# zwu88/TANTE

Hardware: AMD Instinct MI355X
Metric: rollout frames/sec (fwd), TANTE on 256x256 Active Matter (higher is better)
Workload: dtype bf16

## Files before the change

### tante_amd/_lib.py

```python
import ctypes as C
import os

HERE = os.path.dirname(os.path.abspath(__file__))
LIB_PATH = os.environ.get("TANTE_LIB") or os.path.join(HERE, "lib", "libtante_hip.so")

F32, BF16 = 0, 1
INSTNORM_INSTANCE, INSTNORM_RMS = 0, 1
ACT_NONE, ACT_GELU_ERF, ACT_GELU_TANH, ACT_RELU = 0, 1, 2, 3
A_LINEAR, A_PATCH_NHWC, A_PATCH_NCHW = 0, 1, 2
E_LINEAR, E_FILM, E_DECONV_NHWC, E_DECONV_NCHW = 0, 1, 2, 3
W_LINEAR, W_CONV_NHWC, W_DECONV_NHWC, W_DECONV_NCHW = 0, 1, 2, 3
W_LINEAR_T, W_CONV_NHWC_T, W_DECONV_NHWC_T, W_DECONV_NCHW_T = 4, 5, 6, 7

c_i32, c_i64, c_f32, c_vp = C.c_int32, C.c_int64, C.c_float, C.c_void_p


class PackGeom(C.Structure):
    _fields_ = [("n_pad", c_i32), ("k_pad", c_i32), ("nt", c_i32), ("cb", c_i32), ("bytes", c_i64)]


class Gemm(C.Structure):
    _fields_ = [
        ("a", c_vp), ("a_dtype", c_i32), ("a_mode", c_i32), ("M", c_i32), ("K", c_i32),
        ("a_s1", c_i64), ("a_s0", c_i64), ("a_off", c_i64), ("a_n0", c_i32),
# ... 222 lines not shown
    "tante_attention_flash_masked": ([c_vp, c_vp, c_vp, c_i32, c_i32, c_i32, c_i32, c_i32, c_i32, c_vp, c_i64, c_vp, c_f32, C.c_uint64, c_vp], c_i32),
    "tante_attention_flash_masked_bwd": ([c_vp, c_vp, c_vp, c_vp, c_vp, c_i32, c_i32, c_i32, c_i32, c_i32, c_i32, c_vp, c_i64, c_vp, c_f32, C.c_uint64, c_vp], c_i32),
    "tante_head_enc_supported": ([c_i32, c_i32], c_i32),
    "tante_head_enc_stream_bytes": ([c_i32], c_i64),
    "tante_head_enc_ws_bytes": ([c_i64], c_i64),
    "tante_pack_head_enc": ([c_vp] * 6 + [c_i32, c_i32, c_vp, c_vp], c_i32),
    "tante_head_enc_fused": ([c_i32, c_vp, c_vp, c_vp, c_i32, c_i64, c_i64, c_i64, c_i32, c_i32, c_i32, c_i32, c_i32, c_vp, c_i64, c_vp, c_i64,
                             c_vp, c_vp, c_vp, c_i64, c_vp], c_i32),
    "tante_adaptive_tail_supported": ([c_i32] * 6, c_i32),
    "tante_adaptive_rt_stream_bytes": ([c_i32], c_i64),
    "tante_adaptive_ws_bytes": ([c_i32, c_i32, c_i32, c_i32], c_i64),
    "tante_pack_adaptive_rt": ([c_vp] * 6 + [c_i32, c_vp, c_vp], c_i32),
    "tante_adaptive_rt": ([c_i32, c_vp, c_vp, c_vp, c_i32, c_i64, c_i64, c_i64, c_i32, c_i32, c_i32, c_i32, c_f32, c_f32, c_vp, c_i64,
                           c_vp, c_vp, c_vp, c_vp, c_vp, c_vp], c_i32),
    "tante_head_adaptive": ([c_i32, c_vp, c_vp, c_i32, c_i64, c_i64, c_i64, c_i32, c_i32, c_i32, c_i32, c_i32, c_vp, c_vp, c_vp, c_i32, c_vp,
                             c_i32, c_vp, c_i64, c_vp, c_i64, c_vp], c_i32),
    "tante_afno_filter_supported": ([c_i64, c_i32, c_i32, c_i32, c_i32], c_i32),
    "tante_afno_twiddle_floats": ([c_i32, c_i32], c_i64),
    "tante_afno_filter_workspace_bytes": ([c_i64, c_i32, c_i32, c_i32], c_i64),
    "tante_afno_filter": ([c_vp, c_vp, c_i64, c_i32, c_i32, c_i32, c_i32, c_vp, c_vp, c_vp, c_f32, c_vp, c_vp, c_i64, c_vp], c_i32),
    "tante_afno_twiddle_bwd_floats": ([c_i32, c_i32], c_i64),
    "tante_afno_filter_bwd_workspace_bytes": ([c_i64, c_i32, c_i32, c_i32, c_i32], c_i64),
    "tante_afno_filter_bwd": ([c_vp, c_vp, c_i64, c_i32, c_i32, c_i32, c_i32, c_vp, c_vp, c_vp, c_vp, c_f32, c_vp, c_vp, c_vp, c_i32, c_vp, c_vp,
                               c_i64, c_vp], c_i32),
    "tante_groupnorm_supported": ([c_i64, c_i32, c_i32, c_i32], c_i32),
    "tante_groupnorm_workspace_bytes": ([c_i64, c_i32, c_i32, c_i32], c_i64),
    "tante_groupnorm": ([c_vp, c_i64, c_i32, c_i32, c_i32, c_f32, c_vp, c_vp, c_vp, c_i32, c_vp, c_i64, c_vp], c_i32),
    "tante_dpot_filter_supported": ([c_i64, c_i32, c_i32, c_i32, c_i32, c_i32, c_i32], c_i32),
    "tante_dpot_twiddle_floats": ([c_i32, c_i32, c_i32], c_i64),
    "tante_dpot_filter_workspace_bytes": ([c_i64, c_i32, c_i32, c_i32, c_i32, c_i32], c_i64),
    "tante_dpot_filter": ([c_vp, c_vp, c_i64, c_i32, c_i32, c_i32, c_i32, c_i32, c_i32, c_vp, c_vp, c_vp, c_vp, c_vp, c_vp, c_vp, c_i64, c_vp],
                          c_i32),
    "tante_groupnorm_bwd_supported": ([c_i64, c_i32, c_i32, c_i32], c_i32),
    "tante_groupnorm_bwd_workspace_bytes": ([c_i64, c_i32, c_i32, c_i32], c_i64),
    "tante_groupnorm_bwd": ([c_vp, c_i32, c_vp, c_i64, c_i32, c_i32, c_i32, c_f32, c_vp, c_vp, c_vp, c_vp, c_i32, c_vp, c_i64, c_vp], c_i32),
    "tante_dpot_twiddle_bwd_floats": ([c_i32, c_i32, c_i32], c_i64),
    "tante_dpot_filter_bwd_workspace_bytes": ([c_i64, c_i32, c_i32, c_i32, c_i32, c_i32], c_i64),
    "tante_dpot_filter_bwd": ([c_vp, c_vp, c_i64, c_i32, c_i32, c_i32, c_i32, c_i32, c_vp, c_vp, c_vp, c_vp, c_vp, c_vp, c_vp, c_vp, c_vp, c_vp,
                               c_i32, c_vp, c_i64, c_vp], c_i32),
    "tante_instnorm_supported": ([c_i64, c_i32, c_i32], c_i32),
    "tante_instnorm_workspace_bytes": ([c_i64, c_i32, c_i32], c_i64),
    "tante_instnorm": ([c_vp, c_i64, c_i32, c_i32, c_i32, c_f32, c_vp, c_vp, c_i32, c_vp, c_vp, c_vp, c_i32, c_vp, c_i64, c_vp], c_i32),
    "tante_axial_attention_supported": ([c_i64, c_i32, c_i32, c_i32, c_i32], c_i32),
    "tante_axial_attention": ([c_vp, c_i64, c_i32, c_i32, c_i32, c_i32, c_vp, c_vp, c_vp, c_vp, c_f32, c_vp, c_vp], c_i32),
    "tante_time_attention_supported": ([c_i64, c_i32, c_i32, c_i32], c_i32),
    "tante_time_attention": ([c_vp, c_i64, c_i32, c_i32, c_i32, c_vp, c_vp, c_vp, c_vp, c_f32, c_vp, c_vp, c_vp], c_i32),
    "tante_field_stats_supported": ([c_i64, c_i32, c_i32, c_i64], c_i32),
    "tante_field_stats_workspace_bytes": ([c_i64, c_i32, c_i32, c_i64], c_i64),
    "tante_field_stats": ([c_vp, c_i64, c_i32, c_i32, c_i64, c_f32, c_vp, c_vp, c_vp, c_i64, c_vp], c_i32),
    "tante_field_affine_supported": ([c_i64, c_i32, c_i32, c_i64], c_i32),
    "tante_field_affine": ([c_vp, c_vp, c_i64, c_i32, c_i32, c_i64, c_vp, c_vp], c_i32),
    "tante_convnext_block_supported": ([c_i64, c_i32, c_i32, c_i32], c_i32),
    "tante_convnext_stream_bytes": ([c_i32], c_i64),
    "tante_pack_convnext": ([c_vp] * 6 + [c_i32, c_i32, c_vp, c_vp], c_i32),
    "tante_convnext_block": ([c_vp, c_vp, c_vp, c_i64, c_i32, c_i32, c_i32, c_i32, c_f32, c_vp], c_i32),
    "tante_dwconv_ln_supported": ([c_i64, c_i32, c_i32, c_i32], c_i32),
    "tante_dwconv_ln": ([c_vp, c_i64, c_i32, c_i32, c_i32, c_vp, c_vp, c_f32, c_vp, c_vp, c_vp, c_i32, c_vp], c_i32),
    "tante_l2norm_rows_supported": ([c_i64, c_i32], c_i32),
    "tante_l2norm_rows": ([c_vp, c_i64, c_i32, c_f32, c_vp, c_i32, c_vp], c_i32),
    "tante_conv3x3_supported": ([c_i64, c_i32, c_i32, c_i32, c_i32], c_i32),
    "tante_conv3x3": ([c_vp, c_i64, c_i32, c_i32, c_i32, c_i32, c_vp, c_vp, c_i32, c_vp, c_i32, c_vp], c_i32),
    "tante_conv3x3_mfma_supported": ([c_i64, c_i32, c_i32, c_i32, c_i32, c_i32, c_i32], c_i32),
    "tante_conv3x3_pack_bytes": ([c_i32, c_i32, c_i32], c_i64),
    "tante_pack_conv3x3": ([c_vp, c_i32, c_i32, c_i32, c_vp, c_vp], c_i32),
    "tante_conv3x3_mfma": ([c_vp, c_i32, c_vp, c_i32, c_i64, c_i32, c_i32, c_i32, c_i32, c_i32, c_vp, c_vp, c_i32, c_i32, c_i32, c_vp, c_i32, c_vp],
                           c_i32),
    "tante_attn_gate_supported": ([c_i64, c_i32, c_i32, c_i32], c_i32),
    "tante_attn_gate_stream_bytes": ([c_i32, c_i32, c_i32, c_i32], c_i64),
    "tante_pack_attn_gate": ([c_vp, c_vp, c_vp, c_f32, c_i32, c_i32, c_i32, c_i32, c_vp, c_vp], c_i32),
    "tante_attn_gate": ([c_vp, c_vp, c_i64, c_i32, c_i32, c_i32, c_vp, c_i32, c_vp, c_vp], c_i32),
    "tante_uno_block_supported": ([c_i64, c_i32, c_i32, c_i32, c_i32, c_i32, c_i32, c_i32, c_i32, c_i64, c_i64], c_i32),
    "tante_uno_table_floats": ([c_i32, c_i32, c_i32, c_i32, c_i32, c_i32, c_i32], c_i64),
    "tante_uno_table_layout": ([c_i32, c_i32, c_i32, c_i32, c_i32, c_i32, c_i32, c_vp], c_i32),
    "tante_uno_block_workspace_bytes": ([c_i64, c_i32, c_i32, c_i32, c_i32, c_i32, c_i32, c_i32, c_i32, c_i32], c_i64),
    "tante_uno_block": ([c_vp, c_i64, c_i64, c_i32, c_i32, c_i32, c_i32, c_i32, c_i32, c_i32, c_i32, c_vp, c_vp, c_vp, c_vp, c_vp, c_i32, c_vp, c_i64,
                         c_vp, c_i64, c_vp], c_i32),
    "tante_uno_mode_mix_supported": ([c_i64, c_i32, c_i32, c_i32, c_i32], c_i32),
    "tante_uno_mode_mix": ([c_vp, c_vp, c_vp, c_vp, c_i64, c_i32, c_i32, c_i32, c_i32, c_vp], c_i32),
}

LIB_OPTIONS = ("TANTE_ATTN_BWD_HG", "TANTE_ATTN_BWD_NO_SPLIT", "TANTE_ATTN_BWD_VALU", "TANTE_ATTN_FWD_VALU", "TANTE_AXIS_BWD_SMALL_WGS",
               "TANTE_AXIS_BLOCKS", "TANTE_AXIS_BWD_WGS", "TANTE_AXIS_CT", "TANTE_AXIS_FILM", "TANTE_AXIS_GENERIC", "TANTE_AXIS_MFMA", "TANTE_AXIS_NT", "TANTE_AXIS_WGRAD_WGS",
               "TANTE_BLOCK_KERNEL", "TANTE_COLSUM_ROWS", "TANTE_CONV3_FORM","TANTE_CVIT_CHAIN_TOKENS", "TANTE_ENC23_SPLIT", "TANTE_FILM_BWD_ROWS",
               "TANTE_FS_GROUPS", "TANTE_FS_HALF", "TANTE_FS_SKEW", "TANTE_FS_WAVES", "TANTE_GEMM_NO_LITE", "TANTE_GEMM_SMALLM", "TANTE_GEMM_WGS", "TANTE_HEAD_WAVES",
               "TANTE_IM2COL_TILED", "TANTE_RAW_ENCODE_ONE_LAUNCH", "TANTE_RESIZE_TILED", "TANTE_SPECTRAL_BF16OUT", "TANTE_SPECTRAL_DFT", "TANTE_SPECTRAL_X3", "TANTE_WGRAD_DEEP",
               "TANTE_WGRAD_JOBS", "TANTE_WGRAD_JOBS_WGS", "TANTE_WGRAD_NO_SLAB", "TANTE_WGRAD_NO_TR", "TANTE_WGRAD_REDUCE_NY",
               "TANTE_WGRAD_RG", "TANTE_WGRAD_SLAB_WGS", "TANTE_WGRAD_TR_WGS", "TANTE_WGRAD_WGS", "TANTE_XATTN_GPW", "TANTE_XATTN_STREAM", "TANTE_XATTN_VALU",)


_lib = None
ABI_VERSION = 14


def lib():
    global _lib
    if _lib is None:
        if not os.path.exists(LIB_PATH):
            raise RuntimeError(
                f"{LIB_PATH} is missing: build it with `python -m tante_amd.build` "
                "(or __graft_entry__.build()).  tante_amd has no CPU / eager fallback.")
        L = C.CDLL(LIB_PATH)
        for name, (argtypes, restype) in SIGNATURES.items():
            fn = getattr(L, name)
            fn.argtypes = argtypes
            fn.restype = restype
        got = int(L.tante_abi_version())
        if got != ABI_VERSION:
            raise RuntimeError(f"{LIB_PATH}: library ABI {got}, this binding expects {ABI_VERSION} -- a stale build (or a stale variant under "
                               "TANTE_LIB); rebuild with `python -m tante_amd.build`")
        _lib = L
        import warnings
        for k in LIB_OPTIONS:
            v = os.environ.get(k)
            if v is None:
                continue
            try:
                rc = L.tante_set_option(k.encode(), int(v))
            except ValueError:
                warnings.warn(f"{k}={v!r}: library options are integers; ignored")
                continue
            if rc != 0:
                warnings.warn(f"{k}={v}: tante_set_option refused it ({L.tante_last_error().decode(errors='replace')})")
    return _lib


def set_option(name: str, value: int) -> None:
    check(lib().tante_set_option(name.encode(), int(value)), "tante_set_option")


def get_option(name: str, default: int = 0) -> int:
    return int(lib().tante_get_option(name.encode(), int(default)))


def check(rc: int, what: str = ""):
    if rc != 0:
        msg = lib().tante_last_error().decode(errors="replace")
        raise RuntimeError(f"libtante_hip {what} failed (rc={rc}): {msg}")
```

### tante_amd/csrc/block_fused.hip

```cpp
#include "common.hip.h"

#include <stdlib.h>
#include "fused_common.hip.h"
#include "block_sliced.h"

namespace {

constexpr int BIAS_BYTES = 4096;

__device__ __forceinline__ long seq_token(const TanteSeq& q, int s, int l) {
  return (long)(s / q.n_s0) * q.S1 + (long)(s % q.n_s0) * q.S0 + (long)(l / q.n_l0) * q.P1 + (long)(l % q.n_l0) * q.P0;
}

template <int BYTES>
__device__ __forceinline__ void glds_copy(const char* __restrict__ g, char* l, int tid) {
  static_assert(BYTES % 4096 == 0, "tiles are whole LDS-DMA passes");
  const int wave = tid >> 6, lane = tid & 63;
#pragma unroll
  for (int i = 0; i < BYTES / 4096; ++i) {
    const int off = i * 4096 + wave * 1024;
    __builtin_amdgcn_global_load_lds((const __attribute__((address_space(1))) void*)(g + off + lane * 16),
                                     (__attribute__((address_space(3))) void*)(l + off), 16, 0, 0);
  }
}
// ... 632 lines not shown
  if (C != 64 && C != 128 && C != 256) return 0;
  if (hidden != C && hidden != 2 * C) return 0;
  if (hidden > 256 && C == 256) return 0;
  if (L <= 0 || L > 32 || 32 % L) return 0;
  return 1;
}

static int64_t block_ts_stream_bytes(int C, int hidden) {
  const long cpr = C / 8, cprh = hidden / 8;
  return (long)(C / 32) * (96 * cpr * 16 + BIAS_BYTES) + (long)(C / 64 + hidden / 64) * (64 * cpr * 16 + BIAS_BYTES) +
         (long)(C / 64) * (64 * cprh * 16 + BIAS_BYTES);
}

static bool use_fs(int C, int n_head, int hidden, int L, int causal) {
  const int which = tante_opt("TANTE_BLOCK_KERNEL", 0);
  if (!tante_fs_supported(C, n_head, hidden, L, causal)) return false;
  return which == 0 || !block_ts_supported(C, n_head, hidden, L);
}

extern "C" int tante_block_fused_supported(int C, int n_head, int hidden, int L) {
  return block_ts_supported(C, n_head, hidden, L) || tante_fs_supported(C, n_head, hidden, L, 0);
}

extern "C" int64_t tante_block_stream_bytes(int C, int hidden) { return block_ts_stream_bytes(C, hidden) + tante_fs_stream_bytes(C, hidden); }

extern "C" int tante_pack_block(const float* ln1_w, const float* ln1_b, const float* in_w, const float* in_b, const float* out_w,
                                const float* out_b, const float* ln2_w, const float* ln2_b, const float* fc1_w,
                                const float* fc1_b, const float* fc2_w, const float* fc2_b, int C, int hidden,
                                void* block_stream, void* stream) {
  if (!ln1_w || !ln1_b || !in_w || !in_b || !out_w || !out_b || !ln2_w || !ln2_b || !fc1_w || !fc1_b || !fc2_w || !fc2_b ||
      !block_stream)
    TANTE_FAIL(-1, "tante_pack_block: null pointer");
  if (!block_ts_supported(C, C / 32, hidden, 32)) TANTE_FAIL(-2, "tante_pack_block: unsupported C=%d hidden=%d", C, hidden);
  hipLaunchKernelGGL(pack_block_stream_kernel, dim3(C / 32 + 2 * (C / 64) + hidden / 64), dim3(256), 0, (hipStream_t)stream, in_w,
                     in_b, ln1_w, ln1_b, out_w, out_b, fc1_w, fc1_b, ln2_w, ln2_b, fc2_w, fc2_b, C, hidden, (char*)block_stream);
  TANTE_CHECK_LAUNCH();
  if (tante_fs_stream_bytes(C, hidden) > 0) {
    tante_fs_pack(ln1_w, ln1_b, in_w, in_b, out_w, out_b, ln2_w, ln2_b, fc1_w, fc1_b, fc2_w, fc2_b,
                  (char*)block_stream + block_ts_stream_bytes(C, hidden), (hipStream_t)stream);
    TANTE_CHECK_LAUNCH();
  }
  return 0;
}

extern "C" int tante_block_fused_tprop(float* x, const void* block_stream, int C, int n_head, int hidden, const TanteSeq* seq, int causal, float eps,
                                       const float* tprop, void* stream) {
  if (!x || !block_stream || !seq || !tprop) TANTE_FAIL(-1, "tante_block_fused_tprop: null pointer");
  if (seq->L != 4 || !tante_block_fused_supported(C, n_head, hidden, seq->L) || !use_fs(C, n_head, hidden, seq->L, causal))
    TANTE_FAIL(-2, "tante_block_fused_tprop: the feature-sliced kernel at L = 4 only (C=%d heads=%d hidden=%d L=%d)", C, n_head, hidden, seq->L);
  if (((uintptr_t)x % 16) || ((uintptr_t)block_stream % 16)) TANTE_FAIL(-1, "tante_block_fused_tprop: buffers must be 16-byte aligned");
  if (tante_fs_launch(x, (const char*)block_stream + block_ts_stream_bytes(C, hidden), *seq, causal, eps, (hipStream_t)stream, nullptr, tprop) != 0)
    TANTE_FAIL(-2, "tante_block_fused_tprop: too many sequences (%d)", seq->nseq);
  TANTE_CHECK_LAUNCH();
  return 0;
}

extern "C" int tante_block_fused_last_supported(int C, int n_head, int hidden, int L) {
  return C == 256 && n_head == 8 && hidden == 256 && L == 4 && use_fs(C, n_head, hidden, L, 0);
}

extern "C" int tante_block_fused_last(float* x, const void* block_stream, int C, int n_head, int hidden, const TanteSeq* seq, int causal,
                                      float eps, const float* tprop, void* stream) {
  if (!x || !block_stream || !seq) TANTE_FAIL(-1, "tante_block_fused_last: null pointer");
  if (!tante_block_fused_last_supported(C, n_head, hidden, seq->L))
    TANTE_FAIL(-2, "tante_block_fused_last: the feature-sliced kernel at C = 256 / 8 heads / hidden 256 / L = 4 only (C=%d heads=%d hidden=%d L=%d)",
               C, n_head, hidden, seq->L);
  if (((uintptr_t)x % 16) || ((uintptr_t)block_stream % 16)) TANTE_FAIL(-1, "tante_block_fused_last: buffers must be 16-byte aligned");
  if (tante_fs_launch(x, (const char*)block_stream + block_ts_stream_bytes(C, hidden), *seq, causal, eps, (hipStream_t)stream, nullptr, tprop,
                      true) != 0)
    TANTE_FAIL(-2, "tante_block_fused_last: too many sequences (%d)", seq->nseq);
  TANTE_CHECK_LAUNCH();
  return 0;
}

extern "C" int tante_block_fused(float* x, const void* block_stream, int C, int n_head, int hidden, const TanteSeq* seq, int causal,
                                 float eps, void* stream) {
  if (!x || !block_stream || !seq) TANTE_FAIL(-1, "tante_block_fused: null pointer");
  if (!tante_block_fused_supported(C, n_head, hidden, seq->L))
    TANTE_FAIL(-2, "tante_block_fused: unsupported shape C=%d heads=%d hidden=%d L=%d", C, n_head, hidden, seq->L);
  if (((uintptr_t)x % 16) || ((uintptr_t)block_stream % 16)) TANTE_FAIL(-1, "tante_block_fused: buffers must be 16-byte aligned");
  hipStream_t s = (hipStream_t)stream;
  const char* st = (const char*)block_stream;
  if (use_fs(C, n_head, hidden, seq->L, causal)) {
    if (tante_fs_launch(x, st + block_ts_stream_bytes(C, hidden), *seq, causal, eps, s) != 0)
      TANTE_FAIL(-2, "tante_block_fused: too many sequences (%d)", seq->nseq);
    TANTE_CHECK_LAUNCH();
    return 0;
  }
  const int key = (C / 32) * 100 + hidden / 32;
  switch (key) {
    case 202: launch_block<2, 2>(x, st, *seq, causal, eps, s); break;
    case 204: launch_block<2, 4>(x, st, *seq, causal, eps, s); break;
    case 404: launch_block<4, 4>(x, st, *seq, causal, eps, s); break;
    case 408: launch_block<4, 8>(x, st, *seq, causal, eps, s); break;
    case 808: launch_block<8, 8>(x, st, *seq, causal, eps, s); break;
    default: TANTE_FAIL(-2, "tante_block_fused: no instantiation for C=%d hidden=%d", C, hidden);
  }
  TANTE_CHECK_LAUNCH();
  return 0;
}

extern "C" int tante_block_fused_train(const float* x, const void* block_stream, int C, int n_head, int hidden, const TanteSeq* seq, int causal,
                                       float eps, const TanteBlockTrain* tr, void* stream) {
  if (!x || !block_stream || !seq || !tr || !tr->out || !tr->xh1 || !tr->o || !tr->xh2 || !tr->hpre || !tr->act || !tr->st1 ||
      !tr->st2)
    TANTE_FAIL(-1, "tante_block_fused_train: null pointer");
  if (!tante_fs_supported(C, n_head, hidden, seq->L, causal) || seq->L > 64)
    TANTE_FAIL(-2, "tante_block_fused_train: unsupported shape C=%d heads=%d hidden=%d L=%d", C, n_head, hidden, seq->L);
  if (tr->p_drop < 0.0f || tr->p_drop >= 1.0f) TANTE_FAIL(-1, "tante_block_fused_train: dropout probability %f", (double)tr->p_drop);
  const char* st = (const char*)block_stream + block_ts_stream_bytes(C, hidden);
  if (tante_fs_launch((float*)x, st, *seq, causal, eps, (hipStream_t)stream, tr) != 0)
    TANTE_FAIL(-2, "tante_block_fused_train: launch refused (L=%d, %d sequences)", seq->L, seq->nseq);
  TANTE_CHECK_LAUNCH();
  return 0;
}

extern "C" int tante_pack_block_train_multi(const TanteBlockWeights* blocks, int n, int C, int hidden, void* stream) {
  if (!blocks || n <= 0) TANTE_FAIL(-1, "tante_pack_block_train_multi: bad argument");
  if (tante_fs_stream_bytes(C, hidden) == 0) TANTE_FAIL(-2, "tante_pack_block_train_multi: unsupported C=%d hidden=%d", C, hidden);
  for (int g = 0; g < n; g += TANTE_FSP_MAX) {
    const int m = n - g < TANTE_FSP_MAX ? n - g : TANTE_FSP_MAX;
    const float* params[TANTE_FSP_MAX][8];
    char* dst[TANTE_FSP_MAX];
    for (int e = 0; e < m; ++e) {
      const TanteBlockWeights& b = blocks[g + e];
      if (!b.in_w || !b.in_b || !b.out_w || !b.out_b || !b.fc1_w || !b.fc1_b || !b.fc2_w || !b.fc2_b || !b.block_stream)
        TANTE_FAIL(-1, "tante_pack_block_train_multi: null pointer in entry %d", g + e);
      const float* q[8] = {b.in_w, b.in_b, b.out_w, b.out_b, b.fc1_w, b.fc1_b, b.fc2_w, b.fc2_b};
      for (int k = 0; k < 8; ++k) params[e][k] = q[k];
      dst[e] = (char*)b.block_stream + block_ts_stream_bytes(C, hidden);
    }
    tante_fs_pack_folded_multi(params, dst, m, (hipStream_t)stream);
  }
  TANTE_CHECK_LAUNCH();
  return 0;
}

extern "C" int tante_pack_block_train(const float* in_w_folded, const float* in_b_folded, const float* out_w, const float* out_b,
                                      const float* fc1_w_folded, const float* fc1_b_folded, const float* fc2_w, const float* fc2_b, int C,
                                      int hidden, void* block_stream, void* stream) {
  if (!in_w_folded || !in_b_folded || !out_w || !out_b || !fc1_w_folded || !fc1_b_folded || !fc2_w || !fc2_b || !block_stream)
    TANTE_FAIL(-1, "tante_pack_block_train: null pointer");
  if (tante_fs_stream_bytes(C, hidden) == 0) TANTE_FAIL(-2, "tante_pack_block_train: unsupported C=%d hidden=%d", C, hidden);
  tante_fs_pack_folded(in_w_folded, in_b_folded, out_w, out_b, fc1_w_folded, fc1_b_folded, fc2_w, fc2_b,
                       (char*)block_stream + block_ts_stream_bytes(C, hidden), (hipStream_t)stream);
  TANTE_CHECK_LAUNCH();
  return 0;
}
```

### tante_amd/csrc/block_sliced.h

```cpp
#pragma once
#include <hip/hip_runtime.h>
#include <stdint.h>
#include "../../include/tante_hip.h"

int tante_fs_supported(int C, int n_head, int hidden, int L, int causal);
int64_t tante_fs_stream_bytes(int C, int hidden);
void tante_fs_pack(const float* ln1_w, const float* ln1_b, const float* in_w, const float* in_b, const float* out_w, const float* out_b,
                   const float* ln2_w, const float* ln2_b, const float* fc1_w, const float* fc1_b, const float* fc2_w,
                   const float* fc2_b, char* dst, hipStream_t s);
void tante_fs_pack_folded(const float* in_w, const float* in_b, const float* out_w, const float* out_b, const float* fc1_w,
                          const float* fc1_b, const float* fc2_w, const float* fc2_b, char* dst, hipStream_t s);
constexpr int TANTE_FSP_MAX = 12;
void tante_fs_pack_folded_multi(const float* const (*params)[8], char* const* dst, int n, hipStream_t s);
int tante_fs_launch(float* x, const char* stream, const TanteSeq& sq, int causal, float eps, hipStream_t s, const TanteBlockTrain* tr = nullptr,
                    const float* tprop = nullptr, bool lastq = false);
```

### tante_amd/csrc/block_sliced.hip

```cpp
#include "common.hip.h"
#include "fused_common.hip.h"
#include "fs_common.hip.h"
#include "block_sliced.h"

namespace {


struct FsArgs {
  float* x;
  const char* w;
  TanteSeq sq;
  int causal;
  float eps;
  int spw;
  unsigned magic;
  float* out;
  unsigned short *xh1, *qkv, *o, *xh2, *hpre, *act;
  float *st1, *x1, *st2;
  float p_drop;
  unsigned long long seed_attn, seed_out, seed_mlp;
  const unsigned long long* seed_mix;
  unsigned long long* stamps;
  const float* tprop;
  int skew;
};

#ifdef TANTE_ABLATE
#define FS_STAMP(k)                                                                                        \
  do {                                                                                                     \
    if (A.stamps) {                                                                                        \
      unsigned long long t_;                                                                               \
      __builtin_amdgcn_sched_barrier(0);                                                                   \
      asm volatile("s_memtime %0\n\ts_waitcnt lgkmcnt(0)" : "=s"(t_)::"memory");                          \
      __builtin_amdgcn_sched_barrier(0);                                                                   \
      if (lane == 0) A.stamps[((long)vblock * 8 + wave) * 20 + (k)] = t_;                               \
    }                                                                                                      \
  } while (0)
unsigned long long* g_fs_stamps = nullptr;
#else
#define FS_STAMP(k)
#endif

__device__ __forceinline__ void fs_divmod(int a, int n, float rn, int& q, int& r) {
  q = (int)((float)a * rn);
  r = a - q * n;
  if (r >= n) { ++q; r -= n; }
  if (r < 0) { --q; r += n; }
}
struct FsSeqMap {
  float rs0, rl0;
  __device__ __forceinline__ explicit FsSeqMap(const TanteSeq& q) : rs0(__builtin_amdgcn_rcpf((float)q.n_s0)), rl0(__builtin_amdgcn_rcpf((float)q.n_l0)) {}
  __device__ __forceinline__ long token(const TanteSeq& q, int s, int l) const {
    int a, b, c, d;
    fs_divmod(s, q.n_s0, rs0, a, b);
    fs_divmod(l, q.n_l0, rl0, c, d);
    return (long)a * q.S1 + (long)b * q.S0 + (long)c * q.P1 + (long)d * q.P0;
  }
};


struct TpropW {
  float w1c[4], w2c[4];
  f32x4 b1v, b2v;
};
__device__ __forceinline__ void tprop_weights(const float* __restrict__ tp, int lane, TpropW& w) {
#pragma unroll
  for (int a = 0; a < 4; ++a) { w.w1c[a] = tp[4 * (lane & 3) + a]; w.w2c[a] = tp[20 + 4 * (lane & 3) + a]; }
  w.b1v = f32x4{tp[16], tp[17], tp[18], tp[19]};
  w.b2v = f32x4{tp[36], tp[37], tp[38], tp[39]};
}
__device__ __forceinline__ void tprop_apply(const TpropW& w, f32x4 (&xs)[4]) {
  f32x4 hid[4], yy[4];
#pragma unroll
  for (int e = 0; e < 4; ++e) {
    f32x4 h = w.b1v;
#pragma unroll
    for (int a = 0; a < 4; ++a) h = __builtin_amdgcn_mfma_f32_4x4x1f32(w.w1c[a], xs[a][e], h, 0, 0, 0);
    hid[e] = h;
  }
#pragma unroll
  for (int e = 0; e < 4; ++e) hid[e] = gelu_poly4<false>(hid[e]);
#pragma unroll
  for (int e = 0; e < 4; ++e) {
    f32x4 acc = f32x4{xs[0][e], xs[1][e], xs[2][e], xs[3][e]} + w.b2v;
#pragma unroll
    for (int j = 0; j < 4; ++j) acc = __builtin_amdgcn_mfma_f32_4x4x1f32(w.w2c[j], hid[e][j], acc, 0, 0, 0);
    yy[e] = acc;
  }
#pragma unroll
  for (int t = 0; t < 4; ++t) xs[t] = f32x4{yy[0][t], yy[1][t], yy[2][t], yy[3][t]};
}

constexpr int fs_group(int ntt, int nk) {
  int g = 1;
  for (int d = 1; d <= ntt; ++d)
    if (ntt % d == 0 && d * nk <= 8) g = d;
  return g;
}

template <int TPS, int NTT, int NW, bool TRAIN, int G = 1, bool TPROP = false, bool LASTQ = false>
__global__ __launch_bounds__(64 * NW * G, 2) void block_fs_kernel(FsArgs A) {
  static_assert(!TPROP || (TPS == 1 && !TRAIN), "the fused temporal propagator: T letter (L = 4), inference");
  static_assert(!LASTQ || (TPS == 1 && NW == 4 && G == 1 && !TRAIN), "the last-slot form: T letter (L = 4), 4 waves, inference");
  static_assert(G == 1 || (G == 2 && NW == 4), "the paired form is two 4-wave groups");
  constexpr int RT = 16 / NW;
  constexpr int HPW = RT / 2;
  constexpr int FS_PF8 = 3, FS_PF4 = 2;
  constexpr bool TIGHT = (NW == 4 && NTT == 4 && (TRAIN || TPS == 0)) || (NW == 8 && NTT == 8);
  constexpr int PF = (NW == 8 ? FS_PF8 : FS_PF4) - (TIGHT ? 1 : 0);
  constexpr int IMG = 16 * NTT * FS_ROW;
  constexpr int LDS_G = 2 * IMG + 16 * NTT * NW * 8 + FS_BIAS_FLOATS * 4;
  extern __shared__ __attribute__((aligned(16))) char smem_all[];
  const int grp = G == 1 ? 0 : __builtin_amdgcn_readfirstlane((int)threadIdx.x >> 8);
  char* const smem = smem_all + grp * LDS_G;
  char* const bufA = smem;
  char* const bufB = smem + IMG;
  char* const stat = smem + 2 * IMG;
  float* const lbias = (float*)(stat + 16 * NTT * NW * 8);
  const int tid = threadIdx.x & (64 * NW - 1), lane = tid & 63, kk = lane >> 4, l15 = lane & 15;
  const int wave = __builtin_amdgcn_readfirstlane(tid >> 6);
  const int vblock = (int)blockIdx.x * G + grp;
  if constexpr (G == 2) {
    if (grp == 1) __builtin_amdgcn_s_barrier();
  }
  if constexpr (G == 1) {
    if ((__builtin_amdgcn_s_getreg(0x1804) & 1u) == 1u) __builtin_amdgcn_s_setprio(3);
  }
  if constexpr (!TRAIN && G == 1) {
    if (A.skew > 0 && blockIdx.x >= (gridDim.x >> 1)) {
      for (int i = 0; i < A.skew; ++i) __builtin_amdgcn_s_sleep(8);
    }
  }
  float* const x = A.x;
  const unsigned long long smix = (TRAIN && A.seed_mix) ? *A.seed_mix : 0ull;
  const unsigned long long sd_attn = A.seed_attn ^ smix;
  const int L = A.sq.L;
  const int seq0 = vblock * A.spw;
  const int nlive = min(A.spw, A.sq.nseq - seq0) * L;
  const int nslot = A.spw * L;

  const FsW wq = fs_wstream(A.w, (unsigned)((RT * wave) * FS_FRAG + lane * 16));
  u32x4 wb[PF + 1][RT];
  FS_STAMP(0);
#ifdef TANTE_ABLATE
  if (A.stamps && lane == 0) {
    A.stamps[((long)vblock * 8 + wave) * 20 + 16] = __builtin_amdgcn_s_getreg((31 << 11) | 4);
    A.stamps[((long)vblock * 8 + wave) * 20 + 17] = __builtin_amdgcn_s_getreg((31 << 11) | 20);
    A.stamps[((long)vblock * 8 + wave) * 20 + 18] = __builtin_amdgcn_s_memrealtime();
  }
#endif
  int tslot[2];
  {
    const FsSeqMap smap(A.sq);
#pragma unroll
    for (int h = 0; h < (16 * NTT > 64 ? 2 : 1); ++h) {
      const int slot = lane + 64 * h;
      const int s = (int)(((unsigned)slot * A.magic) >> 16), p = slot - s * L;
      tslot[h] = slot < nlive ? (int)smap.token(A.sq, seq0 + s, p) : -1;
    }
  }
  auto tok_of = [&](int slot) { return __shfl(slot < 64 ? tslot[0] : tslot[16 * NTT > 64 ? 1 : 0], slot & 63); };
  for (int i = tid; i < FS_BIAS_FLOATS / 4; i += 64 * NW) *(f32x4*)(lbias + 4 * i) = *(const f32x4*)((const float*)(A.w + FS_W_BYTES) + 4 * i);
  FS_STAMP(1);
  int tokidx[NTT];
#pragma unroll
  for (int tt = 0; tt < NTT; ++tt) tokidx[tt] = tok_of(16 * tt + l15);

  constexpr int CPR = 4 * RT, RPI = 64 / CPR, ROWB = CPR * 16, TILEB = 16 * ROWB;
  constexpr int NSUB = (IMG / NW) / TILEB >= 2 ? 2 : 1;
  static_assert((IMG / NW) >= TILEB, "staging piece too small");
  char* const stg = bufA + wave * (IMG / NW);
  const int rrow = lane / CPR, rchunk = lane % CPR;
  auto srow = [&](int j) { return RPI * j + rrow; };
  auto slice_load = [&](const float* __restrict__ src, f32x4 (&raw)[NTT][RT]) {
#pragma unroll
    for (int tt = 0; tt < NTT; ++tt)
#pragma unroll
      for (int j = 0; j < RT; ++j) {
        const int t = tok_of(16 * tt + srow(j));
        raw[tt][j] = *(const f32x4*)(src + (long)(t < 0 ? 0 : t) * FS_C + 16 * RT * wave + 4 * rchunk);
      }
  };
  auto slice_to_acc = [&](const f32x4 (&raw)[NTT][RT], f32x4 (&acc)[RT][NTT]) {
#pragma unroll
    for (int tt = 0; tt < NTT; ++tt) {
      char* sb = stg + (tt % NSUB) * TILEB;
#pragma unroll
      for (int j = 0; j < RT; ++j) {
        const int r = srow(j);
        *(f32x4*)(sb + r * ROWB + ((rchunk ^ (r & (CPR - 1))) << 4)) = raw[tt][j];
      }
#pragma unroll
// ... 349 lines not shown
      f32x4 o[QG][2];
      static_for<QG>([&](auto qt_c) {
        constexpr int qt = decltype(qt_c)::value;
        constexpr int k0 = TPS > 0 ? ((q0 + qt) / TPS) * TPS : 0;
        constexpr int g0 = k0 / 2, g1 = (k0 + NK - 1) / 2;
        o[qt][0] = o[qt][1] = zero4;
        static_for<g1 - g0 + 1>([&](auto g_c) {
          constexpr int g = g0 + decltype(g_c)::value;
          constexpr int ja = 2 * g - k0, jb = 2 * g + 1 - k0;
          f32x4 pa = zero4, pb = zero4;
          if constexpr (ja >= 0 && ja < NK) pa = sc[qt][ja];
          if constexpr (jb >= 0 && jb < NK) pb = sc[qt][jb];
          const u32x4 pf = pack8(pa, pb);
          o[qt][0] = mfma_bf16(vtf[hh][0][g], pf, o[qt][0]);
          o[qt][1] = mfma_bf16(vtf[hh][1][g], pf, o[qt][1]);
        });
      });
#pragma unroll
      for (int qt = 0; qt < QG; ++qt) {
        const float inv = sum[qt] > 0.0f ? __builtin_amdgcn_rcpf(sum[qt]) : 0.0f;
        const f32x4 o0 = o[qt][0] * inv, o1 = o[qt][1] * inv;
        u32x2 w0, w1;
        w0[0] = pack_bf16x2(o0[0], o0[1]); w0[1] = pack_bf16x2(o0[2], o0[3]);
        w1[0] = pack_bf16x2(o1[0], o1[1]); w1[1] = pack_bf16x2(o1[2], o1[3]);
        *(u32x2*)(bufB + (q0 + qt) * 8192 + wro[2 * hh]) = w0;
        *(u32x2*)(bufB + (q0 + qt) * 8192 + wro[2 * hh + 1]) = w1;
      }
    });
  }
  if constexpr (TRAIN) {
#pragma unroll
    for (int tt = 0; tt < NTT; ++tt) img_rows_store(bufB, tt, A.o, FS_C, 0);
  }

  FS_STAMP(7);
  asm volatile("" ::: "memory");
  f32x4 xraw[NTT][RT];
  fs_wring_prime<3, RT, PF>(wq, wb);
  slice_load(x, xraw);
  FS_STAMP(8);
  __syncthreads();
  FS_STAMP(9);

  f32x4 x1[RT][NTT];
#pragma unroll
  for (int rt = 0; rt < RT; ++rt) {
    const f32x4 bo = *(const f32x4*)(bias + (TRAIN ? 1536 : 256) + 16 * rt);
#pragma unroll
    for (int tt = 0; tt < NTT; ++tt) x1[rt][tt] = bo;
  }
  fs_slice_gemm<3, 48, NTT, RT, false, PF>(wq, wb, bufB, rdo, x1);
  auto drop_add = [&](f32x4 (&acc)[RT][NTT], f32x4 (&res)[RT][NTT], unsigned long long seed) {
    if constexpr (TRAIN) {
      if (A.p_drop > 0.0f) {
        const float ksc = 1.0f / (1.0f - A.p_drop);
#pragma unroll
        for (int tt = 0; tt < NTT; ++tt) {
          const unsigned long long i0 = (unsigned long long)(tokidx[tt] < 0 ? 0 : tokidx[tt]) * FS_C + 16 * RT * wave + 4 * kk;
#pragma unroll
          for (int rt = 0; rt < RT; ++rt) {
            const unsigned k01 = dropout_keep2(seed, i0 + 16 * rt, A.p_drop), k23 = dropout_keep2(seed, i0 + 16 * rt + 2, A.p_drop);
            acc[rt][tt][0] = (k01 & 1u) ? acc[rt][tt][0] * ksc : 0.0f;
            acc[rt][tt][1] = (k01 & 2u) ? acc[rt][tt][1] * ksc : 0.0f;
            acc[rt][tt][2] = (k23 & 1u) ? acc[rt][tt][2] * ksc : 0.0f;
            acc[rt][tt][3] = (k23 & 2u) ? acc[rt][tt][3] * ksc : 0.0f;
          }
        }
      }
    }
#pragma unroll
    for (int rt = 0; rt < RT; ++rt)
#pragma unroll
      for (int tt = 0; tt < NTT; ++tt) acc[rt][tt] += res[rt][tt];
  };
  {
    f32x4 xr[RT][NTT];
    slice_to_acc(xraw, xr);
    drop_add(x1, xr, A.seed_out ^ smix);
  }
  if constexpr (TRAIN) {
    if (A.x1) slice_store(A.x1, x1);
  }
  FS_STAMP(10);
#pragma unroll
  for (int tt = 0; tt < NTT; ++tt) {
    float s = 0.f, q = 0.f;
#pragma unroll
    for (int rt = 0; rt < RT; ++rt)
#pragma unroll
      for (int r = 0; r < 4; ++r) {
        s += x1[rt][tt][r];
        q = fmaf(x1[rt][tt][r], x1[rt][tt][r], q);
      }
    s = rows_sum(s);
    q = rows_sum(q);
    if (kk == 0) *(float2*)(stat + ((16 * tt + l15) * NW + wave) * 8) = make_float2(s, q);
  }
  __syncthreads();
  FS_STAMP(11);
#pragma unroll
  for (int tt = 0; tt < NTT; ++tt) {
    const f32x4* sp = (const f32x4*)(stat + (16 * tt + l15) * NW * 8);
    float s = 0.f, q = 0.f;
#pragma unroll
    for (int j = 0; j < NW / 2; ++j) {
      const f32x4 a = sp[j];
      s += a[0] + a[2];
      q += a[1] + a[3];
    }
    const float mean = s * (1.0f / FS_C);
    const float var = fmaxf(q * (1.0f / FS_C) - mean * mean, 0.0f);
    const float rstd = rsqrtf(var + A.eps);
    const float sh = -mean * rstd;
#pragma unroll
    for (int rt = 0; rt < RT; ++rt) {
      u32x2 o2;
      o2[0] = pack_bf16x2(fmaf(x1[rt][tt][0], rstd, sh), fmaf(x1[rt][tt][1], rstd, sh));
      o2[1] = pack_bf16x2(fmaf(x1[rt][tt][2], rstd, sh), fmaf(x1[rt][tt][3], rstd, sh));
      *(u32x2*)(bufA + tt * 8192 + wro[rt]) = o2;
    }
    if constexpr (TRAIN) {
      img_rows_store(bufA, tt, A.xh2, FS_C, 0);
      if (wave == 0 && kk == 0 && tokidx[tt] >= 0) *(float2*)(A.st2 + 2 * (long)tokidx[tt]) = make_float2(mean, rstd);
    }
  }
  __syncthreads();
  FS_STAMP(12);

  {
    f32x4 h[RT][NTT];
#pragma unroll
    for (int rt = 0; rt < RT; ++rt) {
      const f32x4 b1 = *(const f32x4*)(bias + 512 + 16 * rt);
#pragma unroll
      for (int tt = 0; tt < NTT; ++tt) h[rt][tt] = b1;
    }
    fs_slice_gemm<4, 48, NTT, RT, false, PF>(wq, wb, bufA, rdo, h);
    FS_STAMP(13);
    if constexpr (G == 2) __builtin_amdgcn_s_barrier();
#pragma unroll
    for (int tt = 0; tt < NTT; ++tt) {
      if constexpr (TRAIN) {
#pragma unroll
        for (int rt = 0; rt < RT; ++rt) {
          u32x2 hp;
          hp[0] = pack_bf16x2(h[rt][tt][0], h[rt][tt][1]);
          hp[1] = pack_bf16x2(h[rt][tt][2], h[rt][tt][3]);
          *(u32x2*)(bufB + tt * 8192 + wro[rt]) = hp;
        }
        img_rows_store(bufB, tt, A.hpre, FS_C, 0);
      }
#pragma unroll
      for (int rt = 0; rt < RT; ++rt) {
        const f32x4 g = gelu_poly4<true>(h[rt][tt]);
        u32x2 o2;
        o2[0] = pack_bf16x2(g[0], g[1]);
        o2[1] = pack_bf16x2(g[2], g[3]);
        *(u32x2*)(bufB + tt * 8192 + wro[rt]) = o2;
      }
      if constexpr (TRAIN) img_rows_store(bufB, tt, A.act, FS_C, 0);
    }
  }
  __syncthreads();
  FS_STAMP(14);

  {
    f32x4 y2[TRAIN ? RT : 1][TRAIN ? NTT : 1];
    if constexpr (TRAIN) {
#pragma unroll
      for (int rt = 0; rt < RT; ++rt) {
        const f32x4 b2 = *(const f32x4*)(bias + 768 + 16 * rt);
#pragma unroll
        for (int tt = 0; tt < NTT; ++tt) y2[rt][tt] = b2;
      }
      fs_slice_gemm<5, 48, NTT, RT, false, PF>(wq, wb, bufB, rdo, y2);
      drop_add(y2, x1, A.seed_mlp ^ smix);
#pragma unroll
      for (int rt = 0; rt < RT; ++rt)
#pragma unroll
        for (int tt = 0; tt < NTT; ++tt) x1[rt][tt] = y2[rt][tt];
    } else {
#pragma unroll
      for (int rt = 0; rt < RT; ++rt) {
        const f32x4 b2 = *(const f32x4*)(bias + 768 + 16 * rt);
#pragma unroll
        for (int tt = 0; tt < NTT; ++tt) x1[rt][tt] += b2;
      }
      fs_slice_gemm<5, 48, NTT, RT, false, PF>(wq, wb, bufB, rdo, x1);
// ... 27 lines not shown
    float v[8];
#pragma unroll
    for (int e = 0; e < 8; ++e) {
      const int k = 32 * ks + 8 * kk + e;
      float xv = src[(long)row * C + k];
      if (gamma) xv *= gamma[k];
      v[e] = xv * scale;
    }
    u32x4 o;
    o[0] = pack_bf16x2(v[0], v[1]); o[1] = pack_bf16x2(v[2], v[3]); o[2] = pack_bf16x2(v[4], v[5]); o[3] = pack_bf16x2(v[6], v[7]);
    *(u32x4*)(dst + (long)f * FS_FRAG + lane * 16) = o;
    return;
  }
  __shared__ float bv[FS_C];
  const int n = threadIdx.x;
  if (!be1) {
    float* bias = (float*)(dst + FS_W_BYTES);
    bias[n] = b_in[n] * qscale;
    bias[256 + n] = b_out[n];
    bias[512 + n] = b1[n];
    bias[768 + n] = b2[n];
    bias[1024 + n] = b_in[C + n];
    bias[1280 + n] = b_in[2 * C + n];
    bias[1536 + n] = b_out[n];
    return;
  }
  {
    float s = b_in[2 * C + n];
    for (int k = 0; k < C; ++k) s += w_in[(long)(2 * C + n) * C + k] * be1[k];
    bv[n] = s;
  }
  __syncthreads();
  float* bias = (float*)(dst + FS_W_BYTES);
  {
    float s = b_in[n];
    for (int k = 0; k < C; ++k) s += w_in[(long)n * C + k] * be1[k];
    bias[n] = s * qscale;
  }
  {
    float s = b_out[n];
    for (int c = 0; c < C; ++c) s += w_out[(long)n * C + c] * bv[c];
    bias[256 + n] = s;
  }
  {
    float s = b1[n];
    for (int k = 0; k < C; ++k) s += w1[(long)n * C + k] * be2[k];
    bias[512 + n] = s;
  }
  bias[768 + n] = b2[n];
  {
    float s = b_in[C + n];
    for (int k = 0; k < C; ++k) s += w_in[(long)(C + n) * C + k] * be1[k];
    bias[1024 + n] = s;
  }
  bias[1280 + n] = bv[n];
  bias[1536 + n] = b_out[n];
}
__global__ void fs_pack_kernel(const float* __restrict__ w_in, const float* __restrict__ b_in, const float* __restrict__ g1,
                               const float* __restrict__ be1, const float* __restrict__ w_out, const float* __restrict__ b_out,
                               const float* __restrict__ w1, const float* __restrict__ b1, const float* __restrict__ g2,
                               const float* __restrict__ be2, const float* __restrict__ w2, const float* __restrict__ b2,
                               char* __restrict__ dst) {
  fs_pack_body((int)blockIdx.x, w_in, b_in, g1, be1, w_out, b_out, w1, b1, g2, be2, w2, b2, dst);
}
constexpr int FSP_BLOCKS = FS_W_BYTES / FS_FRAG / 4 + 1;
struct FsPackBatch {
  const float* p[TANTE_FSP_MAX][8];
  char* dst[TANTE_FSP_MAX];
};
__global__ void fs_pack_multi_kernel(FsPackBatch B) {
  const int e = blockIdx.x / FSP_BLOCKS;
  const float* const* q = B.p[e];
  fs_pack_body((int)blockIdx.x - e * FSP_BLOCKS, q[0], q[1], nullptr, nullptr, q[2], q[3], q[4], q[5], nullptr, nullptr, q[6], q[7], B.dst[e]);
}

template <int TPS, int NTT, int NW, bool TRAIN, int G = 1, bool TPROP = false, bool LASTQ = false>
void fs_launch_tt(const FsArgs& A, int nwg, hipStream_t s) {
  constexpr int LDS = G * (2 * 16 * NTT * FS_ROW + 16 * NTT * NW * 8 + FS_BIAS_FLOATS * 4);
  static_assert(LDS <= 160 * 1024, "LDS per workgroup");
  static TantePerDevice attr;
  attr.once([&] { (void)hipFuncSetAttribute((const void*)block_fs_kernel<TPS, NTT, NW, TRAIN, G, TPROP, LASTQ>, hipFuncAttributeMaxDynamicSharedMemorySize, LDS); });
  hipLaunchKernelGGL((block_fs_kernel<TPS, NTT, NW, TRAIN, G, TPROP, LASTQ>), dim3((nwg + G - 1) / G), dim3(64 * NW * G), LDS, s, A);
}
template <int NTT>
void fs_launch_last(const FsArgs& A, int nwg, hipStream_t s) {
  if (A.tprop) fs_launch_tt<1, NTT, 4, false, 1, true, true>(A, nwg, s);
  else fs_launch_tt<1, NTT, 4, false, 1, false, true>(A, nwg, s);
}
template <int TPS, int NTT, int NW>
void fs_launch_t(const FsArgs& A, int nwg, hipStream_t s) {
  if constexpr (NW == 4) {
    if (A.out) return fs_launch_tt<TPS, NTT, NW, true>(A, nwg, s);
    if constexpr (TPS == 1) {
      if (A.tprop) return fs_launch_tt<TPS, NTT, NW, false, 1, true>(A, nwg, s);
    }
    const int groups = tante_opt("TANTE_FS_GROUPS", 0);
    if (groups == 2) return fs_launch_tt<TPS, NTT, NW, false, 2>(A, nwg, s);
  }
  fs_launch_tt<TPS, NTT, NW, false>(A, nwg, s);
}

int fs_waves(int L) {
  const int force8 = tante_opt("TANTE_FS_WAVES", 0) == 8;
  return (force8 || L > 64) ? 8 : 4;
}

}

#ifdef TANTE_ABLATE
extern "C" void tante_fs_set_stamps(void* p) { g_fs_stamps = (unsigned long long*)p; }
#endif

int tante_fs_supported(int C, int n_head, int hidden, int L, int causal) {
  (void)causal;
  return C == FS_C && n_head == 8 && hidden == FS_C && L >= 1 && L <= 128;
}

int64_t tante_fs_stream_bytes(int C, int hidden) { return (C == FS_C && hidden == FS_C) ? FS_W_BYTES + FS_BIAS_FLOATS * 4 : 0; }

void tante_fs_pack(const float* ln1_w, const float* ln1_b, const float* in_w, const float* in_b, const float* out_w, const float* out_b,
                   const float* ln2_w, const float* ln2_b, const float* fc1_w, const float* fc1_b, const float* fc2_w,
                   const float* fc2_b, char* dst, hipStream_t s) {
  hipLaunchKernelGGL(fs_pack_kernel, dim3(FS_W_BYTES / FS_FRAG / 4 + 1), dim3(256), 0, s, in_w, in_b, ln1_w, ln1_b, out_w, out_b, fc1_w,
                     fc1_b, ln2_w, ln2_b, fc2_w, fc2_b, dst);
}

void tante_fs_pack_folded(const float* in_w, const float* in_b, const float* out_w, const float* out_b, const float* fc1_w,
                          const float* fc1_b, const float* fc2_w, const float* fc2_b, char* dst, hipStream_t s) {
  hipLaunchKernelGGL(fs_pack_kernel, dim3(FS_W_BYTES / FS_FRAG / 4 + 1), dim3(256), 0, s, in_w, in_b, (const float*)nullptr,
                     (const float*)nullptr, out_w, out_b, fc1_w, fc1_b, (const float*)nullptr, (const float*)nullptr, fc2_w, fc2_b, dst);
}

void tante_fs_pack_folded_multi(const float* const (*params)[8], char* const* dst, int n, hipStream_t s) {
  FsPackBatch B;
  for (int e = 0; e < n; ++e) {
    for (int k = 0; k < 8; ++k) B.p[e][k] = params[e][k];
    B.dst[e] = dst[e];
  }
  hipLaunchKernelGGL(fs_pack_multi_kernel, dim3((unsigned)(n * FSP_BLOCKS)), dim3(256), 0, s, B);
}

int tante_fs_launch(float* x, const char* stream, const TanteSeq& sq, int causal, float eps, hipStream_t s, const TanteBlockTrain* tr,
                    const float* tprop, bool lastq) {
  if (sq.nseq >= (1 << 23)) return -2;
  if (tprop && (tr || sq.L != 4)) return -5;
  if (lastq && (tr || sq.L != 4)) return -5;
  FsArgs A;
  A.x = x; A.w = stream; A.sq = sq; A.causal = causal; A.eps = eps;
  A.out = nullptr;
  A.seed_mix = nullptr;
  A.tprop = tprop;
  if (tr) {
    if (sq.L > 64) return -4;
    A.out = tr->out; A.xh1 = (unsigned short*)tr->xh1; A.st1 = tr->st1; A.qkv = (unsigned short*)tr->qkv; A.o = (unsigned short*)tr->o;
    A.x1 = tr->x1; A.xh2 = (unsigned short*)tr->xh2; A.st2 = tr->st2; A.hpre = (unsigned short*)tr->hpre; A.act = (unsigned short*)tr->act;
    A.p_drop = tr->p_drop; A.seed_attn = tr->seed_attn; A.seed_out = tr->seed_out; A.seed_mlp = tr->seed_mlp;
    A.seed_mix = tante_seed_mix_ptr();
  }
  A.stamps = nullptr;
#ifdef TANTE_ABLATE
  A.stamps = g_fs_stamps;
#endif
  const int L = sq.L, nw = (tr || tprop || lastq) ? 4 : fs_waves(L);
  A.magic = (65536u + (unsigned)L - 1u) / (unsigned)L;
  int tps = 0;
  if (16 % L == 0) tps = 1;
  else if (!causal && (L == 32 || L == 48 || L == 64)) tps = L / 16;
  const int full = nw == 8 ? 8 : 4, tq = nw == 8 ? 6 : 3;
  const long resident = 256L * (8 / nw);
  auto rounds = [&](int ntt) {
    const int spw = 16 * ntt / L;
    const long nwg = (sq.nseq + spw - 1) / spw;
    return ((nwg + resident - 1) / resident) * ntt;
  };
  int ntt = full;
  if (tps == 3) ntt = tq;
  else if (tps >= 1 && (16 * tq) % L == 0 && (16 * tq) / L >= 1 && (tps == 1 || tq % tps == 0) && rounds(tq) < rounds(full)) ntt = tq;
  if (!tr && nw == 4 && (tps == 1 || tps == 2) && 32 % L == 0 && tante_opt("TANTE_FS_HALF", 1)) {
    const int spw_full = 16 * ntt / L;
    if (((long)sq.nseq + spw_full - 1) / spw_full * 4 <= resident) ntt = 2;
  }
  if (lastq && ntt == tq) ntt = full;
  A.spw = tps ? 16 * ntt / L : (16 * full) / L;
  const int nwg = (sq.nseq + A.spw - 1) / A.spw;
  A.skew = (!tr && nw == 4 && nwg > 256 && nwg <= 512) ? tante_opt("TANTE_FS_SKEW", 0) : 0;
  if (lastq) {
    if (ntt == 2) fs_launch_last<2>(A, nwg, s);
    else fs_launch_last<4>(A, nwg, s);
    return 0;
  }
  const int key = nw * 100 + tps * 10 + ntt;
  switch (key) {
    case 412:
      if (A.tprop) fs_launch_tt<1, 2, 4, false, 1, true>(A, nwg, s);
      else fs_launch_tt<1, 2, 4, false>(A, nwg, s);
      break;
    case 422: fs_launch_tt<2, 2, 4, false>(A, nwg, s); break;
    case 818: fs_launch_t<1, 8, 8>(A, nwg, s); break;
    case 816: fs_launch_t<1, 6, 8>(A, nwg, s); break;
    case 828: fs_launch_t<2, 8, 8>(A, nwg, s); break;
    case 826: fs_launch_t<2, 6, 8>(A, nwg, s); break;
    case 836: fs_launch_t<3, 6, 8>(A, nwg, s); break;
    case 848: fs_launch_t<4, 8, 8>(A, nwg, s); break;
    case 808: fs_launch_t<0, 8, 8>(A, nwg, s); break;
    case 414: fs_launch_t<1, 4, 4>(A, nwg, s); break;
    case 413: fs_launch_t<1, 3, 4>(A, nwg, s); break;
    case 424: fs_launch_t<2, 4, 4>(A, nwg, s); break;
    case 433: fs_launch_t<3, 3, 4>(A, nwg, s); break;
    case 444: fs_launch_t<4, 4, 4>(A, nwg, s); break;
    case 404: fs_launch_t<0, 4, 4>(A, nwg, s); break;
    default: return -3;
  }
  return 0;
}
```

Baseline: 19160.

## Add 8-wave half-tile fused block kernel with pair-chained row statistics

After: 19510 (median of 6 runs). 1.8% higher.

```diff
diff --git a/tante_amd/_lib.py b/tante_amd/_lib.py
--- a/tante_amd/_lib.py
+++ b/tante_amd/_lib.py
@@ -328,7 +328,7 @@
 LIB_OPTIONS = ("TANTE_ATTN_BWD_HG", "TANTE_ATTN_BWD_NO_SPLIT", "TANTE_ATTN_BWD_VALU", "TANTE_ATTN_FWD_VALU", "TANTE_AXIS_BWD_SMALL_WGS",
                "TANTE_AXIS_BLOCKS", "TANTE_AXIS_BWD_WGS", "TANTE_AXIS_CT", "TANTE_AXIS_FILM", "TANTE_AXIS_GENERIC", "TANTE_AXIS_MFMA", "TANTE_AXIS_NT", "TANTE_AXIS_WGRAD_WGS",
                "TANTE_BLOCK_KERNEL", "TANTE_COLSUM_ROWS", "TANTE_CONV3_FORM","TANTE_CVIT_CHAIN_TOKENS", "TANTE_ENC23_SPLIT", "TANTE_FILM_BWD_ROWS",
-               "TANTE_FS_GROUPS", "TANTE_FS_HALF", "TANTE_FS_SKEW", "TANTE_FS_WAVES", "TANTE_GEMM_NO_LITE", "TANTE_GEMM_SMALLM", "TANTE_GEMM_WGS", "TANTE_HEAD_WAVES",
+               "TANTE_FS_GROUPS", "TANTE_FS_HALF", "TANTE_FS_HALF8", "TANTE_FS_SKEW", "TANTE_FS_WAVES", "TANTE_GEMM_NO_LITE", "TANTE_GEMM_SMALLM", "TANTE_GEMM_WGS", "TANTE_HEAD_WAVES",
                "TANTE_IM2COL_TILED", "TANTE_RAW_ENCODE_ONE_LAUNCH", "TANTE_RESIZE_TILED", "TANTE_SPECTRAL_BF16OUT", "TANTE_SPECTRAL_DFT", "TANTE_SPECTRAL_X3", "TANTE_WGRAD_DEEP",
                "TANTE_WGRAD_JOBS", "TANTE_WGRAD_JOBS_WGS", "TANTE_WGRAD_NO_SLAB", "TANTE_WGRAD_NO_TR", "TANTE_WGRAD_REDUCE_NY",
                "TANTE_WGRAD_RG", "TANTE_WGRAD_SLAB_WGS", "TANTE_WGRAD_TR_WGS", "TANTE_WGRAD_WGS", "TANTE_XATTN_GPW", "TANTE_XATTN_STREAM", "TANTE_XATTN_VALU",)
diff --git a/tante_amd/csrc/block_fused.hip b/tante_amd/csrc/block_fused.hip
--- a/tante_amd/csrc/block_fused.hip
+++ b/tante_amd/csrc/block_fused.hip
@@ -738,7 +738,8 @@
   hipStream_t s = (hipStream_t)stream;
   const char* st = (const char*)block_stream;
   if (use_fs(C, n_head, hidden, seq->L, causal)) {
-    if (tante_fs_launch(x, st + block_ts_stream_bytes(C, hidden), *seq, causal, eps, s) != 0)
+    const int half8 = tante_fs_half8_launch(x, st + block_ts_stream_bytes(C, hidden), *seq, causal, eps, s);
+    if (half8 < 0 || (half8 == 0 && tante_fs_launch(x, st + block_ts_stream_bytes(C, hidden), *seq, causal, eps, s) != 0))
       TANTE_FAIL(-2, "tante_block_fused: too many sequences (%d)", seq->nseq);
     TANTE_CHECK_LAUNCH();
     return 0;
diff --git a/tante_amd/csrc/block_sliced.h b/tante_amd/csrc/block_sliced.h
--- a/tante_amd/csrc/block_sliced.h
+++ b/tante_amd/csrc/block_sliced.h
@@ -12,5 +12,6 @@
                           const float* fc1_b, const float* fc2_w, const float* fc2_b, char* dst, hipStream_t s);
 constexpr int TANTE_FSP_MAX = 12;
 void tante_fs_pack_folded_multi(const float* const (*params)[8], char* const* dst, int n, hipStream_t s);
+int tante_fs_half8_launch(float* x, const char* stream, const TanteSeq& sq, int causal, float eps, hipStream_t s);
 int tante_fs_launch(float* x, const char* stream, const TanteSeq& sq, int causal, float eps, hipStream_t s, const TanteBlockTrain* tr = nullptr,
                     const float* tprop = nullptr, bool lastq = false);
diff --git a/tante_amd/csrc/block_sliced.hip b/tante_amd/csrc/block_sliced.hip
--- a/tante_amd/csrc/block_sliced.hip
+++ b/tante_amd/csrc/block_sliced.hip
@@ -98,16 +98,19 @@
   return g;
 }
 
-template <int TPS, int NTT, int NW, bool TRAIN, int G = 1, bool TPROP = false, bool LASTQ = false>
+template <int TPS, int NTT, int NW, bool TRAIN, int G = 1, bool TPROP = false, bool LASTQ = false, bool PAIR = false>
 __global__ __launch_bounds__(64 * NW * G, 2) void block_fs_kernel(FsArgs A) {
   static_assert(!TPROP || (TPS == 1 && !TRAIN), "the fused temporal propagator: T letter (L = 4), inference");
   static_assert(!LASTQ || (TPS == 1 && NW == 4 && G == 1 && !TRAIN), "the last-slot form: T letter (L = 4), 4 waves, inference");
   static_assert(G == 1 || (G == 2 && NW == 4), "the paired form is two 4-wave groups");
+  static_assert(!PAIR || (NW == 8 && NTT == 2 && G == 1 && !TRAIN && !TPROP && !LASTQ), "pair-chained statistics: 8 waves on 2 tiles, inference");
+  constexpr int SNW = PAIR ? NW / 2 : NW;
   constexpr int RT = 16 / NW;
   constexpr int HPW = RT / 2;
   constexpr int FS_PF8 = 3, FS_PF4 = 2;
   constexpr bool TIGHT = (NW == 4 && NTT == 4 && (TRAIN || TPS == 0)) || (NW == 8 && NTT == 8);
-  constexpr int PF = (NW == 8 ? FS_PF8 : FS_PF4) - (TIGHT ? 1 : 0);
+  constexpr int FS_PFH = 3;
+  constexpr int PF = PAIR ? FS_PFH : (NW == 8 ? FS_PF8 : FS_PF4) - (TIGHT ? 1 : 0);
   constexpr int IMG = 16 * NTT * FS_ROW;
   constexpr int LDS_G = 2 * IMG + 16 * NTT * NW * 8 + FS_BIAS_FLOATS * 4;
   extern __shared__ __attribute__((aligned(16))) char smem_all[];
@@ -623,28 +626,61 @@
     if (A.x1) slice_store(A.x1, x1);
   }
   FS_STAMP(10);
-#pragma unroll
-  for (int tt = 0; tt < NTT; ++tt) {
-    float s = 0.f, q = 0.f;
-#pragma unroll
-    for (int rt = 0; rt < RT; ++rt)
-#pragma unroll
-      for (int r = 0; r < 4; ++r) {
-        s += x1[rt][tt][r];
-        q = fmaf(x1[rt][tt][r], x1[rt][tt][r], q);
-      }
-    s = rows_sum(s);
-    q = rows_sum(q);
-    if (kk == 0) *(float2*)(stat + ((16 * tt + l15) * NW + wave) * 8) = make_float2(s, q);
+  if constexpr (PAIR) {
+    auto stat_chain = [&](int tt, float& s, float& q) {
+#pragma unroll
+      for (int rt = 0; rt < RT; ++rt)
+#pragma unroll
+        for (int r = 0; r < 4; ++r) {
+          s += x1[rt][tt][r];
+          q = fmaf(x1[rt][tt][r], x1[rt][tt][r], q);
+        }
+    };
+    float2* const hand = (float2*)(smem + LDS_G) + (wave >> 1) * (NTT * 64) + lane;
+    if ((wave & 1) == 0) {
+#pragma unroll
+      for (int tt = 0; tt < NTT; ++tt) {
+        float s = 0.f, q = 0.f;
+        stat_chain(tt, s, q);
+        hand[64 * tt] = make_float2(s, q);
+      }
+    }
+    __syncthreads();
+    if ((wave & 1) == 1) {
+#pragma unroll
+      for (int tt = 0; tt < NTT; ++tt) {
+        const float2 h = hand[64 * tt];
+        float s = h.x, q = h.y;
+        stat_chain(tt, s, q);
+        s = rows_sum(s);
+        q = rows_sum(q);
+        if (kk == 0) *(float2*)(stat + ((16 * tt + l15) * SNW + (wave >> 1)) * 8) = make_float2(s, q);
+      }
+    }
+  } else {
+#pragma unroll
+    for (int tt = 0; tt < NTT; ++tt) {
+      float s = 0.f, q = 0.f;
+#pragma unroll
+      for (int rt = 0; rt < RT; ++rt)
+#pragma unroll
+        for (int r = 0; r < 4; ++r) {
+          s += x1[rt][tt][r];
+          q = fmaf(x1[rt][tt][r], x1[rt][tt][r], q);
+        }
+      s = rows_sum(s);
+      q = rows_sum(q);
+      if (kk == 0) *(float2*)(stat + ((16 * tt + l15) * NW + wave) * 8) = make_float2(s, q);
+    }
   }
   __syncthreads();
   FS_STAMP(11);
 #pragma unroll
   for (int tt = 0; tt < NTT; ++tt) {
-    const f32x4* sp = (const f32x4*)(stat + (16 * tt + l15) * NW * 8);
+    const f32x4* sp = (const f32x4*)(stat + (16 * tt + l15) * SNW * 8);
     float s = 0.f, q = 0.f;
 #pragma unroll
-    for (int j = 0; j < NW / 2; ++j) {
+    for (int j = 0; j < SNW / 2; ++j) {
       const f32x4 a = sp[j];
       s += a[0] + a[2];
       q += a[1] + a[3];
@@ -838,6 +874,13 @@
   attr.once([&] { (void)hipFuncSetAttribute((const void*)block_fs_kernel<TPS, NTT, NW, TRAIN, G, TPROP, LASTQ>, hipFuncAttributeMaxDynamicSharedMemorySize, LDS); });
   hipLaunchKernelGGL((block_fs_kernel<TPS, NTT, NW, TRAIN, G, TPROP, LASTQ>), dim3((nwg + G - 1) / G), dim3(64 * NW * G), LDS, s, A);
 }
+template <int TPS>
+void fs_launch_half8(const FsArgs& A, int nwg, hipStream_t s) {
+  constexpr int LDS = 2 * 16 * 2 * FS_ROW + 16 * 2 * 8 * 8 + FS_BIAS_FLOATS * 4 + 4 * 2 * 64 * 8;
+  static TantePerDevice attr;
+  attr.once([&] { (void)hipFuncSetAttribute((const void*)block_fs_kernel<TPS, 2, 8, false, 1, false, false, true>, hipFuncAttributeMaxDynamicSharedMemorySize, LDS); });
+  hipLaunchKernelGGL((block_fs_kernel<TPS, 2, 8, false, 1, false, false, true>), dim3(nwg), dim3(512), LDS, s, A);
+}
 template <int NTT>
 void fs_launch_last(const FsArgs& A, int nwg, hipStream_t s) {
   if (A.tprop) fs_launch_tt<1, NTT, 4, false, 1, true, true>(A, nwg, s);
@@ -894,6 +937,33 @@
     B.dst[e] = dst[e];
   }
   hipLaunchKernelGGL(fs_pack_multi_kernel, dim3((unsigned)(n * FSP_BLOCKS)), dim3(256), 0, s, B);
+}
+
+int tante_fs_half8_launch(float* x, const char* stream, const TanteSeq& sq, int causal, float eps, hipStream_t s) {
+  if (sq.nseq >= (1 << 23)) return -2;
+  const int L = sq.L;
+  if (sq.nseq < 1 || L < 1 || 32 % L != 0 || (L == 32 && causal) || fs_waves(L) != 4) return 0;
+  if (!tante_opt("TANTE_FS_HALF", 1) || !tante_opt("TANTE_FS_HALF8", 1)) return 0;
+  auto nwg_at = [&](int ntt) { return ((long)sq.nseq + 16 * ntt / L - 1) / (16 * ntt / L); };
+  auto rounds = [&](int ntt) { return ((nwg_at(ntt) + 511) / 512) * ntt; };
+  const int ntt_full = (L != 32 && rounds(3) < rounds(4)) ? 3 : 4;
+  if (nwg_at(ntt_full) * 4 > 512) return 0;
+  FsArgs A;
+  A.x = x; A.w = stream; A.sq = sq; A.causal = causal; A.eps = eps;
+  A.out = nullptr;
+  A.seed_mix = nullptr;
+  A.tprop = nullptr;
+  A.stamps = nullptr;
+#ifdef TANTE_ABLATE
+  A.stamps = g_fs_stamps;
+#endif
+  A.magic = (65536u + (unsigned)L - 1u) / (unsigned)L;
+  A.spw = 32 / L;
+  A.skew = 0;
+  const int nwg = (int)nwg_at(2);
+  if (L == 32) fs_launch_half8<2>(A, nwg, s);
+  else fs_launch_half8<1>(A, nwg, s);
+  return 1;
 }
 
 int tante_fs_launch(float* x, const char* stream, const TanteSeq& sq, int causal, float eps, hipStream_t s, const TanteBlockTrain* tr,
```
